# uberalex974/Reinforcement-Learning

Measured on AMD Instinct MI355X. Metric: env-steps/sec (whole node) at 32768 arenas; PPO wall-clock per 1M steps, higher is better.
Workload: dtype f32

## Files before the change

### include/rlgpu_core.h

```cpp
#ifndef RLGPU_CORE_H
#define RLGPU_CORE_H

#ifdef __cplusplus
extern "C" {
#endif

enum rlgpu_status {
    RLGPU_OK = 0,
    RLGPU_ERR_INVALID_ARG = -1,
    RLGPU_ERR_HIP = -2,
    RLGPU_ERR_OOM = -3,
    RLGPU_ERR_STATE = -4,
    RLGPU_ERR_UNSUPPORTED = -5
};

const char* rlgpu_last_error(void);

int rlgpu_abi_version(void);

int rlgpu_device_count(void);

#ifdef __cplusplus
}
#endif
#endif
```

### reinforcement-learning_amd/host/learner.cpp

```cpp
#include "learner.hpp"

#include <algorithm>
#include <chrono>
#include <cmath>
#include <cstdio>
#include <cstring>

#include "../csrc/common.hpp"
#include "../csrc/learner_kernels.hpp"

namespace {
constexpr int OBS = RLGPU_OBS, ACT = RLGPU_ACTIONS;
using clk = std::chrono::steady_clock;
double secs(clk::time_point a, clk::time_point b) { return std::chrono::duration<double>(b - a).count(); }

inline void hipCheck(hipError_t e, const char* what) {
    if (e != hipSuccess) throw rlgpu::Error(RLGPU_ERR_HIP, std::string(what) + ": " + hipGetErrorString(e));
}

inline uint64_t splitmix64(uint64_t x) {
    x += 0x9E3779B97F4A7C15ull;
    x = (x ^ (x >> 30)) * 0xBF58476D1CE4E5B9ull;
    x = (x ^ (x >> 27)) * 0x94D049BB133111EBull;
    return x ^ (x >> 31);
}
}

namespace RLGC {

EnvSetGPU::EnvSetGPU(const rlgpu_envset_config& cfg, hipStream_t stream) : stream_(stream) {
    RlgpuCheck(rlgpu_envset_create(&cfg, &h_), "EnvSet");
    RlgpuCheck(rlgpu_envset_buffers_get(h_, &state_), "EnvSet buffers");
}
EnvSetGPU::~EnvSetGPU() {
    if (h_) rlgpu_envset_destroy(h_);
}
void EnvSetGPU::StepFirstHalf(bool) { RlgpuCheck(rlgpu_envset_step_first_half(h_, stream_), "StepFirstHalf"); }
void EnvSetGPU::StepSecondHalf(const int32_t* d_actions, bool async) {
    RlgpuCheck(rlgpu_envset_step_second_half(h_, d_actions, stream_), "StepSecondHalf");
    if (!async) Sync();
}
void EnvSetGPU::Step(const int32_t* d_actions, const rlgpu_step_outputs* out) {
    RlgpuCheck(rlgpu_envset_step(h_, d_actions, 1, out, stream_), "EnvSet step");
}
void EnvSetGPU::Sync() { RlgpuCheck(rlgpu_envset_sync(h_, stream_), "Sync"); }
void EnvSetGPU::Reset() { RlgpuCheck(rlgpu_envset_reset(h_, stream_), "Reset"); }
void EnvSetGPU::ResetArenas(const uint8_t* d_mask) {
    RlgpuCheck(rlgpu_envset_reset_arenas(h_, d_mask, stream_), "ResetArena");
}

}

namespace GGL {

void WelfordStat::Increment(const float* xs, int64_t n) {
    for (int64_t i = 0; i < n; i++) {
        double delta = (double)xs[i] - mean;
        double deltaN = delta / (double)(count + 1);
        mean += deltaN;
        m2 += delta * deltaN * (double)count;
        count++;
    }
}
double WelfordStat::GetSTD() const {
    if (count < 2) return 1.0;
    double var = m2 / (double)(count - 1);
    if (var <= 0) var = 1.0;
    return std::sqrt(var);
}

void MomentsMeanStd(const double* m, float* out) {
    const double mean = m[0] / m[2];
    double var = (m[1] - m[0] * mean) / (m[2] - 1);
    if (!(var > 0)) var = 0;
    out[0] = (float)mean;
    out[1] = (float)std::sqrt(var);
}

std::vector<std::pair<int64_t, int64_t>> BatchRanges(int64_t expSize, int64_t batchSize, bool overbatching) {
    std::vector<std::pair<int64_t, int64_t>> out;
    if (expSize <= 0 || batchSize <= 0) return out;
    for (int64_t start = 0; start < expSize; start += batchSize) {
        int64_t end = start + batchSize;
        if (end + batchSize > expSize && overbatching) end = expSize;
        if (end > expSize || end - start <= 0) break;
        out.emplace_back(start, end);
        if (end == expSize) break;
    }
    return out;
}

template <class T>
void DevArray<T>::Reserve(int64_t n, hipStream_t s, bool keep) {
    if (n <= cap) return;
    const int64_t ncap = std::max<int64_t>(n, cap + cap / 2);
    T* q = nullptr;
    hipCheck(hipMalloc((void**)&q, (size_t)ncap * sizeof(T) + 16), "DevArray alloc");
    if (keep && p && cap > 0) hipCheck(hipMemcpyAsync(q, p, (size_t)cap * sizeof(T), hipMemcpyDeviceToDevice, s), "DevArray copy");
    if (p) {
        hipCheck(hipStreamSynchronize(s), "sync");
        (void)hipFree(p);
    }
    p = q;
    cap = ncap;
}
template <class T>
void DevArray<T>::Free() {
    if (p) (void)hipFree(p);
    p = nullptr;
    cap = 0;
}

void ExperienceBuffer::Allocate(int T_, int P_, int W_, bool rollout_outputs) {
    T = T_;
    P = P_;
    W = W_;
    auto A = [&](size_t bytes) {
        void* p = nullptr;
        hipCheck(hipMalloc(&p, bytes + 16), "ExperienceBuffer alloc");
        hipCheck(hipMemset(p, 0, bytes + 16), "ExperienceBuffer memset");
        allocs.push_back(p);
        return p;
    };
    const size_t TP = (size_t)T * P, T1P = (size_t)(T + 1) * P;
    const size_t OP = rollout_outputs ? TP : (size_t)P, O1P = rollout_outputs ? T1P : (size_t)P;
    v.obs = (float*)A(T1P * W * 4);
    v.masks = (uint8_t*)A(T1P * ACT);
    v.actions = (int32_t*)A(TP * 4);
    v.logp = (float*)A(TP * 4);
    v.rewards = (float*)A(TP * 4);
    v.terms = (int8_t*)A(TP);
    v.trunc_obs = (float*)A(OP * W * 4);
    v.values = (float*)A(O1P * 4);
    v.trunc_vals = (float*)A(OP * 4);
    v.adv = (float*)A(OP * 4);
    v.target = (float*)A(OP * 4);
    v.ret = (float*)A(OP * 4);
    v.T = T;
    v.P = P;
    v.obs_width = W;
}
void ExperienceBuffer::Free() {
    for (void* p : allocs) (void)hipFree(p);
    allocs.clear();
}

PPOLearnerGPU::PPOLearnerGPU(const rlgpu_ppo_config& cfg, hipStream_t stream) : stream_(stream) {
    RlgpuCheck(rlgpu_ppo_create(&cfg, &h_), "PPOLearner");
    float* params = nullptr;
    RlgpuCheck(rlgpu_ppo_buffers(h_, &params, &grads_, &nparams_), "PPOLearner buffers");
    hipCheck(hipMalloc((void**)&adv_stats_, 2 * sizeof(float)), "adv stats");
    hipCheck(hipMalloc((void**)&metrics_, RLGPU_NUM_METRICS * sizeof(float)), "metrics");
    hipCheck(hipMemset(metrics_, 0, RLGPU_NUM_METRICS * sizeof(float)), "metrics");
    RlgpuCheck(rlgpu_ppo_init_params(h_, cfg.seed, stream_), "init params");
}
PPOLearnerGPU::~PPOLearnerGPU() {
    if (adv_stats_) (void)hipFree(adv_stats_);
    if (metrics_) (void)hipFree(metrics_);
    if (h_) rlgpu_ppo_destroy(h_);
}
void PPOLearnerGPU::InferActions(const float* d_obs, const uint8_t* d_masks, int n, bool det, uint64_t step,
                                 int32_t* d_actions, float* d_logp, const uint8_t* d_old_rows) {
    if (d_old_rows)
        RlgpuCheck(rlgpu_ppo_infer_actions_mixed(h_, d_obs, d_masks, n, det, step, d_old_rows, d_actions, d_logp, stream_),
                   "InferActions (old version)");
    else
        RlgpuCheck(rlgpu_ppo_infer_actions(h_, d_obs, d_masks, n, det, step, d_actions, d_logp, stream_), "InferActions");
}
void PPOLearnerGPU::InferCritic(const float* d_obs, int64_t n, float* d_values) {
    RlgpuCheck(rlgpu_ppo_infer_critic(h_, d_obs, n, d_values, stream_), "InferCritic");
}
void PPOLearnerGPU::AdvantageStats(const float* d_adv, int64_t n) {
    RlgpuCheck(rlgpu_mean_std(d_adv, n, adv_stats_, stream_), "advantage stats");
}
void PPOLearnerGPU::Minibatch(const float* d_obs, const uint8_t* d_masks, const int32_t* d_actions, const float* d_logp,
                              const float* d_adv, const float* d_target, const int32_t* d_index, int64_t start, int n,
                              int64_t batch) {
    RlgpuCheck(rlgpu_ppo_minibatch(h_, d_obs, d_masks, d_actions, d_logp, d_adv, d_target, d_index, start, n, batch,
                                   adv_stats_, metrics_, stream_),
               "Learn minibatch");
    minibatches++;
}
void PPOLearnerGPU::OptimizerStep() { RlgpuCheck(rlgpu_ppo_optimizer_step(h_, metrics_, stream_), "optimizer step"); }

template <class T>
T* Learner::Alloc(size_t count) {
    void* p = nullptr;
    hipCheck(hipMalloc(&p, count * sizeof(T) + 16), "Learner alloc");
    allocs_.push_back(p);
    return (T*)p;
}
void Learner::Release(void* p) {
    for (auto& q : allocs_)
        if (q == p) {
            (void)hipFree(q);
            q = allocs_.back();
            allocs_.pop_back();
            return;
        }
}

Learner::Learner(const rlgpu_learner_config& cfg, const rlgpu_collective* coll, hipStream_t stream)
    : s_(stream), cfg_(cfg) {
    RLGPU_REQUIRE(cfg.num_arenas > 0 && cfg.rollout_len > 0 && cfg.epochs > 0 && cfg.mini_batch_size > 0,
                  "Learner: num_arenas, rollout_len, epochs and mini_batch_size must be > 0");
    RLGPU_REQUIRE(cfg.world >= 1 && cfg.rank >= 0 && cfg.rank < cfg.world, "Learner: bad rank / world");
    RLGPU_REQUIRE(cfg.world == 1 || (coll && coll->allreduce_sum_f32 && coll->allreduce_sum_f64 && coll->allgather_f32),
                  "Learner: world > 1 needs a complete rlgpu_collective");
    RLGPU_REQUIRE(cfg.return_samples >= 0, "Learner: return_samples must be >= 0");
    if (coll) {
        coll_ = *coll;
        hasColl_ = cfg.world > 1;
    }
    std::memset(&stats, 0, sizeof(stats));
    const int T = cfg.rollout_len, N = cfg.num_arenas, P = 4 * N;
    rlgpu_envset_config ec{};
    ec.num_arenas = N;
    ec.tick_skip = cfg.tick_skip;
    ec.action_delay = cfg.action_delay;
    ec.seed = cfg.seed * 1000003ull;
    ec.arena_offset = cfg.rank * N;
    ec.save_rewards = 1;
    ec.max_episode_steps = (int32_t)(cfg.max_episode_duration * (120.0f / (float)cfg.tick_skip));
    ec.mesh_tris = cfg.mesh_tris;
    ec.mesh_ntris = cfg.mesh_ntris;
    ec.mesh_objects = cfg.mesh_objects;
    ec.mesh_object_ntris = cfg.mesh_object_ntris;
    ec.rewards = cfg.rewards;
    ec.n_rewards = cfg.n_rewards;
    ec.terminals = cfg.terminals;
    ec.n_terminals = cfg.n_terminals;
    ec.arith = cfg.arith;
    env_ = new RLGC::EnvSetGPU(ec, s_);
    RlgpuCheck(rlgpu_envset_enable_step_metrics(env_->handle(), 1), "step metrics");
    RlgpuCheck(rlgpu_envset_set_output_only(env_->handle(), 1), "output-only rows");
    K_ = cfg.frame_stack > 1 ? cfg.frame_stack : 1;
    RLGPU_REQUIRE(K_ <= 16, "Learner: frame_stack must be <= 16");
    const int W = OBS * K_;
    rlgpu_ppo_config pc{};
    pc.obs_size = W;
    pc.num_actions = ACT;
    std::memcpy(pc.policy_layers, cfg.policy_layers, sizeof(pc.policy_layers));
    pc.n_policy_layers = cfg.n_policy_layers;
    std::memcpy(pc.critic_layers, cfg.critic_layers, sizeof(pc.critic_layers));
    pc.n_critic_layers = cfg.n_critic_layers;
    std::memcpy(pc.shared_layers, cfg.shared_layers, sizeof(pc.shared_layers));
    pc.n_shared_layers = cfg.n_shared_layers;
    RLGPU_REQUIRE(cfg.activation >= RLGPU_ACT_LEAKY_RELU && cfg.activation <= RLGPU_ACT_TANH,
                  "Learner: activation must be RLGPU_ACT_LEAKY_RELU, _RELU, _SIGMOID or _TANH");
    RLGPU_REQUIRE(cfg.no_layer_norm == 0 || cfg.no_layer_norm == 1, "Learner: no_layer_norm must be 0 or 1");
    RLGPU_REQUIRE(cfg.optimizer == RLGPU_OPT_ADAMW || cfg.optimizer == RLGPU_OPT_ADAM,
                  "Learner: optimizer must be RLGPU_OPT_ADAMW or RLGPU_OPT_ADAM");
    pc.layer_norm = cfg.no_layer_norm ? 0 : 1;
    pc.activation = cfg.activation;
    pc.leaky_slope = 0.01f;
    pc.policy_lr = cfg.policy_lr;
    pc.critic_lr = cfg.critic_lr;
    pc.beta1 = 0.9f;
    pc.beta2 = 0.999f;
    pc.eps = 1e-8f;
    pc.weight_decay = cfg.optimizer == RLGPU_OPT_ADAM ? 0.f : 1e-2f;
    pc.clip_range = cfg.clip_range;
    pc.entropy_scale = cfg.entropy_scale;
    pc.max_grad_norm = 0.5f;
    const int64_t TP = (int64_t)T * P;
    const int64_t rowsCap = cfg.experience_mode == RLGPU_EXP_TRAJECTORIES ? (int64_t)cfg.mini_batch_size : TP;
    pc.max_rows = (int32_t)std::max<int64_t>(std::min<int64_t>(cfg.mini_batch_size, rowsCap), std::min<int64_t>(P, 65536));
    pc.seed = cfg.seed;
    pc.sample_row_offset = (int64_t)cfg.rank * P;
    pc.train_gemm = cfg.train_gemm;
    pc.infer_fp16 = cfg.infer_fp16;
    pc.policy_temperature = cfg.policy_temperature;
    pc.mask_entropy = cfg.mask_entropy;
    ppo_ = new PPOLearnerGPU(pc, s_);
    if (hasColl_) {
        float* params = nullptr;
        float* g = nullptr;
        int64_t n = 0;
        RlgpuCheck(rlgpu_ppo_buffers(ppo_->handle(), &params, &g, &n), "buffers");
        if (cfg.rank != 0) hipCheck(hipMemsetAsync(params, 0, n * sizeof(float), s_), "broadcast");
        hipCheck(hipStreamSynchronize(s_), "sync");
        if (coll_.allreduce_sum_f32(coll_.user, params, n) != 0)
            throw rlgpu::Error(RLGPU_ERR_STATE, "Learner: parameter broadcast failed");
        RlgpuCheck(rlgpu_ppo_refresh_half(ppo_->handle(), s_), "refresh half");
    }
    if (trajMode()) {
        RLGPU_REQUIRE(ec.max_episode_steps > 0, "Learner: experience_mode 1 needs max_episode_duration > 0");
        TrajectoryStore& J = traj;
        J.maxLen = ec.max_episode_steps;
        const int64_t total = cfg.ts_per_itr > 0 ? cfg.ts_per_itr : (int64_t)T * P * cfg.world;
        J.tsPerItr = (total + cfg.world - 1) / cfg.world;
        const int64_t perStep = P;
        J.Tmax = cfg.experience_capacity > 0 ? cfg.experience_capacity
                                              : (int)(J.maxLen + 2 * ((J.tsPerItr + perStep - 1) / perStep) + 64);
        RLGPU_REQUIRE(J.Tmax > J.maxLen + 1, "Learner: experience_capacity must exceed the max episode length + 1");
        exp_.Allocate(J.Tmax, P, W, false);
        J.start = Alloc<int32_t>(P);
        J.len = Alloc<int32_t>(P);
        J.trnew = Alloc<int32_t>(P);
        J.counters = Alloc<int64_t>(lk::kTcCount);
        hipCheck(hipMemset(J.start, 0, (size_t)P * 4), "traj start");
        hipCheck(hipMemset(J.len, 0, (size_t)P * 4), "traj len");
        hipCheck(hipHostMalloc((void**)&J.hcounters, lk::kTcCount * sizeof(int64_t)), "pinned counters");
        if (K_ > 1) J.truncStage = Alloc<float>((size_t)P * W);
        const int64_t rc = 4 * (int64_t)P;
        for (auto* a : {&J.rp, &J.rstart, &J.rlen, &J.rcode, &J.rtidx}) a->Reserve(rc, s_);
        J.roff.Reserve(rc, s_);
        J.truncObs.Reserve(4 * (int64_t)P * W, s_);
    } else {
        exp_.Allocate(T, P, W);
    }
    const rlgpu_envset_buffers& st = env_->state();
    if (K_ > 1) {
        hist_ = Alloc<float>((size_t)(K_ - 1) * P * OBS);
        lk::stack_frames(st.obs, nullptr, nullptr, hist_, K_, P, OBS, exp_.v.obs, nullptr, s_);
    } else {
        hipCheck(hipMemcpyAsync(exp_.v.obs, st.obs, (size_t)P * OBS * 4, hipMemcpyDeviceToDevice, s_), "obs0");
    }
    hipCheck(hipMemcpyAsync(exp_.v.masks, st.action_masks, (size_t)P * ACT, hipMemcpyDeviceToDevice, s_), "masks0");
    std::vector<uint8_t> team(P);
    for (int k = 0; k < 2; k++) {
        oldRows_[k] = Alloc<uint8_t>(P);
        for (int p = 0; p < P; p++) team[p] = (uint8_t)(p % 2 == k);
        hipCheck(hipMemcpy(oldRows_[k], team.data(), P, hipMemcpyHostToDevice), "old rows");
    }
    trainRows_ = Alloc<int32_t>((size_t)TP / 2 + 1);
    perm_ = Alloc<int32_t>(TP);
    permRows_ = Alloc<int32_t>(TP);
    badv_ = Alloc<float>(TP);
    permCap_ = TP;
    truncRows_ = Alloc<int32_t>(TP);
    truncCount_ = Alloc<int32_t>(1);
    selBytes_ = lk::select_trunc_scratch_bytes(TP);
    selScratch_ = Alloc<char>(selBytes_);
    sampleIdx_ = Alloc<int64_t>((size_t)std::max(1, cfg.return_samples));
    samples_ = Alloc<float>((size_t)std::max(1, cfg.return_samples));
    ends_ = Alloc<int32_t>(P);
    hostEnds_.assign(P, -1);
    mom_ = (double*)Alloc<char>(4 * sizeof(double) + lk::moments_scratch_bytes());
    clipSums_ = Alloc<float>(2);
    hipCheck(hipStreamSynchronize(s_), "Learner init");
}

Learner::~Learner() {
    if (s_) (void)hipStreamSynchronize(s_);
    for (auto s : gs_) {
        (void)hipStreamSynchronize(s);
        (void)hipStreamDestroy(s);
    }
    for (auto e : gsEnd_) (void)hipEventDestroy(e);
    if (gsStart_) (void)hipEventDestroy(gsStart_);
    for (auto e : ev_) (void)hipEventDestroy(e);
    for (void* p : allocs_) (void)hipFree(p);
    if (truncObsC_) (void)hipFree(truncObsC_);
    if (truncValC_) (void)hipFree(truncValC_);
    if (traj.hcounters) (void)hipHostFree(traj.hcounters);
    for (auto* a : {&traj.rp, &traj.rstart, &traj.rlen, &traj.rcode, &traj.rtidx, &traj.cActs}) a->Free();
    traj.roff.Free();
    for (auto* a : {&traj.truncObs, &traj.truncVals, &traj.cObs, &traj.cLogp, &traj.cRews, &traj.cVals, &traj.cAdv,
                    &traj.cTarget, &traj.cRet})
        a->Free();
    traj.cMasks.Free();
    traj.cTerms.Free();
    exp_.Free();
    delete ppo_;
    delete env_;
}

int Learner::CollectGroups() const {
    const int want = cfg_.collect_groups > 0 ? cfg_.collect_groups : 1;
    if (want <= 1 || hook_ || K_ > 1 || trajMode() || !rlgpu_ppo_fused_infer(ppo_->handle(), 0)) return 1;
    if (cfg_.num_arenas % (4 * want) != 0) return 1;
    return want;
}

void Learner::CollectGrouped(int G) {
    const int T = exp_.T, P = exp_.P, W = exp_.W;
    const rlgpu_rollout_view& v = exp_.v;
    const uint8_t* old = OldRows();
    const int Na = cfg_.num_arenas / G, Pg = 4 * Na;
    if ((int)gs_.size() != G) {
        for (auto s : gs_) (void)hipStreamDestroy(s);
        for (auto e : gsEnd_) (void)hipEventDestroy(e);
        gs_.assign(G, nullptr);
        gsEnd_.assign(G, nullptr);
        for (int g = 0; g < G; g++) {
            hipCheck(hipStreamCreateWithFlags(&gs_[g], hipStreamNonBlocking), "group stream");
            hipCheck(hipEventCreateWithFlags(&gsEnd_[g], hipEventDisableTiming), "group event");
        }
        if (!gsStart_) hipCheck(hipEventCreateWithFlags(&gsStart_, hipEventDisableTiming), "group event");
    }
    if (envTiming_) EnsureEvents((size_t)2 * T * G);
    hipCheck(hipEventRecord(gsStart_, s_), "group start");
    for (int g = 0; g < G; g++) hipCheck(hipStreamWaitEvent(gs_[g], gsStart_, 0), "group wait");
    rlgpu_ppo* ph = ppo_->handle();
    rlgpu_envset* eh = env_->handle();
    for (int t = 0; t < T; t++) {
        const size_t r = (size_t)t * P;
        for (int g = 0; g < G; g++) {
            const size_t p0 = (size_t)g * Pg, a = r + p0;
            RlgpuCheck(rlgpu_ppo_infer_actions_rows(ph, v.obs + a * W, v.masks + a * ACT, Pg, (int64_t)p0,
                                                    cfg_.deterministic != 0, (uint64_t)stats.rng_step,
                                                    old ? old + p0 : nullptr, v.actions + a, v.logp + a, gs_[g]),
                       "InferActions (group)");
            rlgpu_step_outputs o{v.obs + (a + P) * OBS, v.masks + (a + P) * ACT, v.rewards + a, v.terms + a,
                                 v.trunc_obs + a * OBS};
            if (envTiming_) hipCheck(hipEventRecord(ev_[2 * ((size_t)t * G + g)], gs_[g]), "event");
            RlgpuCheck(rlgpu_envset_step_range(eh, g * Na, Na, v.actions + a, 1, &o, gs_[g]), "EnvSet step (group)");
            if (envTiming_) hipCheck(hipEventRecord(ev_[2 * ((size_t)t * G + g) + 1], gs_[g]), "event");
        }
        stats.rng_step++;
    }
    for (int g = 0; g < G; g++) {
        hipCheck(hipEventRecord(gsEnd_[g], gs_[g]), "group end");
        hipCheck(hipStreamWaitEvent(s_, gsEnd_[g], 0), "group join");
    }
}

void Learner::Collect() {
    if (trajMode()) {
        CollectTrajectories();
        return;
    }
    if (const int G = CollectGroups(); G > 1) {
        collectGroupsUsed_ = G;
        CollectGrouped(G);
        return;
    }
    collectGroupsUsed_ = 1;
    const int T = exp_.T, P = exp_.P, W = exp_.W;
    const rlgpu_rollout_view& v = exp_.v;
    if (envTiming_) EnsureEvents((size_t)2 * T);
    for (int t = 0; t < T; t++) {
        const size_t r = (size_t)t * P;
        ActAndStep(r, r + P, v.trunc_obs + r * OBS, v.trunc_obs + r * W, envTiming_ ? &ev_[2 * t] : nullptr);
    }
}

void Learner::ActAndStep(size_t row, size_t next, float* trunc, float* truncStacked, hipEvent_t* timing) {
    const int P = exp_.P, W = exp_.W;
    const rlgpu_rollout_view& v = exp_.v;
    const rlgpu_envset_buffers& st = env_->state();
    ppo_->InferActions(v.obs + row * W, v.masks + row * ACT, P, cfg_.deterministic != 0, (uint64_t)stats.rng_step,
                       v.actions + row, v.logp + row, OldRows());
    stats.rng_step++;
    rlgpu_step_outputs o{K_ > 1 ? nullptr : v.obs + next * OBS, v.masks + next * ACT, v.rewards + row, v.terms + row,
                         K_ > 1 ? nullptr : trunc};
    if (timing) hipCheck(hipEventRecord(timing[0], s_), "event");
    StepEnv(v.actions + row, o);
    if (timing) hipCheck(hipEventRecord(timing[1], s_), "event");
    if (K_ > 1) lk::stack_frames(st.obs, st.trunc_obs, v.terms + row, hist_, K_, P, OBS, v.obs + next * W, truncStacked, s_);
}

void Learner::EnsureEvents(size_t count) {
    if (ev_.size() >= count) return;
    for (auto e : ev_) (void)hipEventDestroy(e);
    ev_.assign(count, nullptr);
    for (auto& e : ev_) hipCheck(hipEventCreate(&e), "event");
}

void Learner::StepEnv(const int32_t* d_actions, const rlgpu_step_outputs& o) {
    if (!hook_) {
        env_->Step(d_actions, &o);
        return;
    }
    rlgpu_envset* e = env_->handle();
    const rlgpu_envset_buffers& st = env_->state();
    const int P = st.num_players;
    rlgpu_step_outputs pre{nullptr, nullptr, nullptr, o.terminals, nullptr};
    RlgpuCheck(rlgpu_envset_step(e, d_actions, 0, &pre, s_), "EnvSet step (hooked)");
    hipCheck(hipStreamSynchronize(s_), "sync");
    if (hook_(hookUser_, RLGPU_HOOK_AFTER_STEP) != 0)
        throw rlgpu::Error(RLGPU_ERR_STATE, std::string("Learner: step hook failed: ") + rlgpu_last_error());
    lk::host_step_finish(st.terminals, o.terminals, st.rewards, o.rewards, st.obs, st.trunc_obs, o.trunc_obs, P, OBS, s_);
    RlgpuCheck(rlgpu_envset_reset(e, s_), "EnvSet reset (hooked)");
    hipCheck(hipStreamSynchronize(s_), "sync");
    if (hook_(hookUser_, RLGPU_HOOK_AFTER_RESET) != 0)
        throw rlgpu::Error(RLGPU_ERR_STATE, std::string("Learner: step hook failed: ") + rlgpu_last_error());
    if (o.obs) hipCheck(hipMemcpyAsync(o.obs, st.obs, (size_t)P * OBS * 4, hipMemcpyDeviceToDevice, s_), "obs append");
    if (o.masks) hipCheck(hipMemcpyAsync(o.masks, st.action_masks, (size_t)P * ACT, hipMemcpyDeviceToDevice, s_), "mask append");
}

void Learner::Consume() {
    if (trajMode()) {
        ConsumeTrajectories();
        return;
    }
    const int T = exp_.T, P = exp_.P;
    const int64_t TP = (int64_t)T * P;
    const rlgpu_rollout_view& v = exp_.v;
    ppo_->InferCritic(v.obs, TP + P, v.values);
    lk::select_trunc(v.terms, TP, selScratch_, selBytes_, truncRows_, truncCount_, s_);
    int32_t ntr = 0;
    hipCheck(hipMemcpyAsync(&ntr, truncCount_, sizeof(int32_t), hipMemcpyDeviceToHost, s_), "trunc count");
    hipCheck(hipStreamSynchronize(s_), "sync");
    if (ntr > 0) {
        if (ntr > truncCap_) {
            if (truncObsC_) (void)hipFree(truncObsC_);
            if (truncValC_) (void)hipFree(truncValC_);
            truncCap_ = std::max<int64_t>(ntr, 2 * truncCap_);
            hipCheck(hipMalloc((void**)&truncObsC_, (size_t)truncCap_ * exp_.W * 4), "trunc obs");
            hipCheck(hipMalloc((void**)&truncValC_, (size_t)truncCap_ * 4), "trunc vals");
        }
        lk::gather_rows(v.trunc_obs, exp_.W, truncRows_, ntr, truncObsC_, s_);
        ppo_->InferCritic(truncObsC_, ntr, truncValC_);
        lk::scatter_f32(truncValC_, truncRows_, ntr, v.trunc_vals, s_);
    }
    const float std_ = (float)returnStat.GetSTD();
    RlgpuCheck(rlgpu_gae_rollout(v.rewards, v.terms, v.values, v.trunc_vals, v.values + TP, T, P, cfg_.gamma,
                                 cfg_.gae_lambda, std_, cfg_.reward_clip_range, v.adv, v.target, v.ret, nullptr, s_),
               "GAE");
    const int k = cfg_.return_samples;
    if (k <= 0) return;
    lk::last_ends(v.terms, T, P, ends_, s_);
    hipCheck(hipMemcpyAsync(hostEnds_.data(), ends_, (size_t)P * sizeof(int32_t), hipMemcpyDeviceToHost, s_), "ends");
    hipCheck(hipStreamSynchronize(s_), "sync");
    if (oldTeam_ >= 0)
        for (int p = oldTeam_; p < P; p += 2) hostEnds_[p] = -1;
    if (!hasColl_) {
        std::vector<int64_t> idx(k);
        int32_t m = 0;
        RlgpuCheck(rlgpu_sample_finished_rows(cfg_.seed, 0, stats.iteration, hostEnds_.data(), P, k, idx.data(), &m),
                   "return samples");
        FeedReturnStat(v.ret, idx, m);
        return;
    }
    const int world = cfg_.world;
    std::vector<float> mine((size_t)P), all((size_t)P * world);
    for (int p = 0; p < P; p++) mine[p] = (float)hostEnds_[p];
    if (coll_.allgather_f32(coll_.user, mine.data(), P, all.data()) != 0)
        throw rlgpu::Error(RLGPU_ERR_STATE, "Learner: trajectory-end all-gather failed");
    std::vector<int32_t> gends((size_t)P * world);
    for (size_t i = 0; i < gends.size(); i++) gends[i] = (int32_t)all[i];
    const int64_t GP = (int64_t)P * world;
    std::vector<int64_t> gidx(k), idx;
    std::vector<int32_t> slot;
    int32_t m = 0;
    RlgpuCheck(rlgpu_sample_finished_rows(cfg_.seed, 0, stats.iteration, gends.data(), (int32_t)GP, k, gidx.data(), &m),
               "return samples");
    for (int32_t i = 0; i < m; i++) {
        const int64_t t = gidx[i] / GP, gp = gidx[i] % GP;
        if (gp / P == cfg_.rank) {
            idx.push_back(t * P + (gp - (int64_t)cfg_.rank * P));
            slot.push_back(i);
        }
    }
    std::vector<float> hs(std::max<size_t>(idx.size(), 1));
    if (!idx.empty()) {
        hipCheck(hipMemcpyAsync(sampleIdx_, idx.data(), idx.size() * sizeof(int64_t), hipMemcpyHostToDevice, s_),
                 "sample idx");
        lk::gather_samples(v.ret, sampleIdx_, (int32_t)idx.size(), samples_, s_);
        hipCheck(hipMemcpyAsync(hs.data(), samples_, idx.size() * sizeof(float), hipMemcpyDeviceToHost, s_), "samples");
        hipCheck(hipStreamSynchronize(s_), "sync");
    }
    std::vector<double> draw((size_t)std::max(m, 1), 0.0);
    for (size_t j = 0; j < idx.size(); j++) draw[slot[j]] = (double)hs[j];
    if (m > 0 && coll_.allreduce_sum_f64(coll_.user, draw.data(), m) != 0)
        throw rlgpu::Error(RLGPU_ERR_STATE, "Learner: return-sample all-reduce failed");
    std::vector<float> got((size_t)std::max(m, 1));
    for (int32_t i = 0; i < m; i++) got[i] = (float)draw[i];
    returnStat.Increment(got.data(), m);
}

void Learner::FeedReturnStat(const float* d_ret, const std::vector<int64_t>& idx, int32_t m) {
    const int k = cfg_.return_samples;
    std::vector<float> hs((size_t)std::max(m, 1));
    if (m > 0) {
        hipCheck(hipMemcpyAsync(sampleIdx_, idx.data(), m * sizeof(int64_t), hipMemcpyHostToDevice, s_), "sample idx");
        lk::gather_samples(d_ret, sampleIdx_, m, samples_, s_);
        hipCheck(hipMemcpyAsync(hs.data(), samples_, m * sizeof(float), hipMemcpyDeviceToHost, s_), "samples");
        hipCheck(hipStreamSynchronize(s_), "sync");
    }
    if (hasColl_) {
        std::vector<float> mine((size_t)k + 1, 0.f), all((size_t)(k + 1) * cfg_.world);
        mine[0] = (float)m;
        std::copy(hs.begin(), hs.begin() + m, mine.begin() + 1);
        if (coll_.allgather_f32(coll_.user, mine.data(), k + 1, all.data()) != 0)
            throw rlgpu::Error(RLGPU_ERR_STATE, "Learner: return-sample all-gather failed");
        for (int r = 0; r < cfg_.world; r++) {
            const float* blk = all.data() + (size_t)r * (k + 1);
            returnStat.Increment(blk + 1, (int64_t)blk[0]);
        }
    } else {
        returnStat.Increment(hs.data(), m);
    }
}

void Learner::AllReduceGrads(int epoch, int batch) {
    if (!hasColl_ && !gradHook_) return;
    hipCheck(hipStreamSynchronize(s_), "sync");
    if (hasColl_ && coll_.allreduce_sum_f32(coll_.user, ppo_->grads(), ppo_->num_params()) != 0)
        throw rlgpu::Error(RLGPU_ERR_STATE, "Learner: gradient all-reduce failed");
    if (gradHook_ && gradHook_(gradHookUser_, ppo_->grads(), ppo_->num_params(), epoch, batch) != 0)
        throw rlgpu::Error(RLGPU_ERR_STATE, "Learner: the gradient hook failed");
}

void Learner::BatchAdvantageStats(const float* d_adv, const int32_t* d_idx, int64_t n) {
    if (!hasColl_) {
        if (d_idx) {
            NeedLearnRows(n, "the batch-advantage gather");
            lk::gather_f32(d_adv, d_idx, n, badv_, s_);
            ppo_->AdvantageStats(badv_, n);
        } else {
            ppo_->AdvantageStats(d_adv, n);
        }
        return;
    }
    lk::moments_f64(d_adv, d_idx, n, mom_ + 4, mom_, s_);
    double m[3];
    hipCheck(hipMemcpyAsync(m, mom_, sizeof(m), hipMemcpyDeviceToHost, s_), "moments");
    hipCheck(hipStreamSynchronize(s_), "sync");
    if (coll_.allreduce_sum_f64(coll_.user, m, 3) != 0)
        throw rlgpu::Error(RLGPU_ERR_STATE, "Learner: advantage-moment all-reduce failed");
    float st[2];
    MomentsMeanStd(m, st);
    hipCheck(hipMemcpyAsync(ppo_->adv_stats(), st, sizeof(st), hipMemcpyHostToDevice, s_), "adv stats");
    hipCheck(hipStreamSynchronize(s_), "sync");
}

void Learner::NeedLearnRows(int64_t n, const char* what) const {
    if (n > permCap_)
        throw rlgpu::Error(RLGPU_ERR_INVALID_ARG, std::string("Learner: ") + what + " needs " + std::to_string(n) +
                                                      " rows of learn scratch, " + std::to_string(permCap_) + " reserved");
}

void Learner::ReserveLearnRows(int64_t M) {
    if (M <= permCap_) return;
    const int64_t cap = std::max<int64_t>(M, permCap_ + permCap_ / 2);
    hipCheck(hipStreamSynchronize(s_), "sync");
    for (void* p : {(void*)perm_, (void*)permRows_, (void*)badv_}) Release(p);
    perm_ = Alloc<int32_t>(cap);
    permRows_ = Alloc<int32_t>(cap);
    badv_ = Alloc<float>(cap);
    permCap_ = cap;
}

void Learner::Learn() {
    const int T = exp_.T, P = exp_.P;
    rlgpu_rollout_view v = exp_.v;
    const bool rows = oldTeam_ >= 0 && !trajMode();
    int64_t M = rows ? (int64_t)T * (P / 2) : (int64_t)T * P;
    if (trajMode()) {
        M = traj.nrows;
        v.obs = traj.cObs.p;
        v.masks = traj.cMasks.p;
        v.actions = traj.cActs.p;
        v.logp = traj.cLogp.p;
        v.adv = traj.cAdv.p;
        v.target = traj.cTarget.p;
        if (M <= 0 && !hasColl_) return;
    }
    ReserveLearnRows(M);
    int64_t globalM = M * cfg_.world;
    if (trajMode() && hasColl_) {
        double m = (double)M;
        if (coll_.allreduce_sum_f64(coll_.user, &m, 1) != 0)
            throw rlgpu::Error(RLGPU_ERR_STATE, "Learner: batch-size all-reduce failed");
        globalM = (int64_t)m;
    }
    const int64_t batch = cfg_.batch_size > 0 ? cfg_.batch_size : globalM;
    const int64_t localBatch = cfg_.batch_size > 0 ? std::max<int64_t>(1, cfg_.batch_size / cfg_.world) : M;
    std::vector<std::pair<int64_t, int64_t>> trajRanges;
    if (trajMode() && hasColl_) {
        for (auto [g0, g1] : BatchRanges(globalM, batch, cfg_.overbatching != 0))
            trajRanges.emplace_back(globalM ? g0 * M / globalM : 0, globalM ? g1 * M / globalM : 0);
        if (trajRanges.empty()) trajRanges.emplace_back(0, 0);
    }
    if (rows) lk::train_rows(T, P, 1 - oldTeam_, trainRows_, s_);
    for (int epoch = 0; epoch < cfg_.epochs; epoch++) {
        NeedLearnRows(M, "the shuffle");
        RlgpuCheck(rlgpu_permutation(M, cfg_.seed + (uint64_t)cfg_.rank, (uint64_t)(stats.iteration * cfg_.epochs + epoch),
                                     perm_, s_),
                   "shuffle");
        const int32_t* order = perm_;
        if (rows) {
            NeedLearnRows(M, "the team row selection");
            if (M > (int64_t)T * (P / 2)) throw rlgpu::Error(RLGPU_ERR_INVALID_ARG, "Learner: team rows exceed T * P / 2");
            lk::compose(trainRows_, perm_, M, permRows_, s_);
            order = permRows_;
        }
        const auto ranges = trajMode() && hasColl_ ? trajRanges : BatchRanges(M, localBatch, cfg_.overbatching != 0);
        int bi = 0;
        for (auto [b0, b1] : ranges) {
            const bool whole = !rows && b0 == 0 && b1 == M;
            BatchAdvantageStats(v.adv, whole ? nullptr : order + b0, b1 - b0);
            for (int64_t s0 = b0; s0 < b1; s0 += cfg_.mini_batch_size) {
                const int n = (int)std::min<int64_t>(cfg_.mini_batch_size, b1 - s0);
                ppo_->Minibatch(v.obs, v.masks, v.actions, v.logp, v.adv, v.target, order, s0, n, batch);
            }
            AllReduceGrads(epoch, bi++);
            ppo_->OptimizerStep();
        }
    }
}

void Learner::FinishIteration() {
    const int T = exp_.T, P = exp_.P;
    const rlgpu_rollout_view& v = exp_.v;
    const size_t W = (size_t)exp_.W;
    const int64_t realPlayers = oldTeam_ < 0 ? P : P / 2;
    stats.iteration++;
    if (trajMode()) {
        stats.total_steps += (int64_t)traj.steps * realPlayers * cfg_.world;
        return;
    }
    hipCheck(hipMemcpyAsync(v.obs, v.obs + (size_t)T * P * W, (size_t)P * W * 4, hipMemcpyDeviceToDevice, s_), "obs");
    hipCheck(hipMemcpyAsync(v.masks, v.masks + (size_t)T * P * ACT, (size_t)P * ACT, hipMemcpyDeviceToDevice, s_), "masks");
    stats.total_steps += (int64_t)T * realPlayers * cfg_.world;
}

lk::TrajRecs TrajectoryStore::Records() const { return {rp.p, rstart.p, rlen.p, rcode.p, rtidx.p, roff.p}; }

void Learner::CollectTrajectories() {
    TrajectoryStore& J = traj;
    const int P = exp_.P, W = exp_.W, Tm = J.Tmax;
    const rlgpu_rollout_view& v = exp_.v;
    const rlgpu_envset_buffers& st = env_->state();
    const uint8_t* track = oldTeam_ >= 0 ? oldRows_[1 - oldTeam_] : nullptr;
    if (J.lastOldTeam >= 0) lk::traj_restart(oldRows_[J.lastOldTeam], P, (int)(J.step % Tm), J.start, J.len, s_);
    J.lastOldTeam = oldTeam_;
    hipCheck(hipMemsetAsync(J.counters, 0, lk::kTcCount * sizeof(int64_t), s_), "traj counters");
    J.firstStep = J.step;
    J.steps = 0;
    J.nrec = J.ntrunc = J.nrows = 0;
    for (;;) {
        const int64_t need = std::max(J.nrec, J.ntrunc) + P;
        if (J.rp.cap < need) {
// ... 399 lines not shown
```

### reinforcement-learning_amd/host/learner.hpp

```cpp
#pragma once
#include <hip/hip_runtime.h>

#include <cstdint>
#include <stdexcept>
#include <string>
#include <utility>
#include <vector>

#include "../../include/rlgpu_env.h"
#include "../../include/rlgpu_gae.h"
#include "../../include/rlgpu_learner.h"
#include "../../include/rlgpu_ppo.h"

namespace RLGC {

inline void RlgpuCheck(int st, const char* what) {
    if (st != RLGPU_OK) throw std::runtime_error(std::string(what) + ": " + rlgpu_last_error());
}

class EnvSetGPU {
public:
    EnvSetGPU(const rlgpu_envset_config& cfg, hipStream_t stream);
    ~EnvSetGPU();
    EnvSetGPU(const EnvSetGPU&) = delete;
    EnvSetGPU& operator=(const EnvSetGPU&) = delete;

    void StepFirstHalf(bool async = true);
    void StepSecondHalf(const int32_t* d_actions, bool async);
    void Step(const int32_t* d_actions, const rlgpu_step_outputs* out);
    void Sync();
    void Reset();
    void ResetArenas(const uint8_t* d_mask);

    rlgpu_envset* handle() const { return h_; }
    const rlgpu_envset_buffers& state() const { return state_; }

private:
    rlgpu_envset* h_ = nullptr;
    rlgpu_envset_buffers state_{};
    hipStream_t stream_;
};

}

namespace lk {
struct TrajRecs;
}

namespace GGL {

using RLGC::RlgpuCheck;

struct WelfordStat {
    int64_t count = 0;
    double mean = 0, m2 = 0;
    void Increment(const float* xs, int64_t n);
    double GetMean() const { return count < 2 ? 0.0 : mean; }
    double GetSTD() const;
};

void MomentsMeanStd(const double* m3, float* out2);

std::vector<std::pair<int64_t, int64_t>> BatchRanges(int64_t expSize, int64_t batchSize, bool overbatching);

struct ExperienceBuffer {
    int T = 0, P = 0, W = 0;
    rlgpu_rollout_view v{};
    std::vector<void*> allocs;
    void Allocate(int T, int P, int W, bool rollout_outputs = true);
    void Free();
};

template <class T>
struct DevArray {
    T* p = nullptr;
    int64_t cap = 0;
    void Reserve(int64_t n, hipStream_t s, bool keep = false);
    void Free();
};

struct TrajectoryStore {
    int Tmax = 0, maxLen = 0;
    int64_t tsPerItr = 0;
    int64_t step = 0;
    int64_t firstStep = 0;
    int steps = 0;
    int lastOldTeam = -1;
    int32_t *start = nullptr, *len = nullptr, *trnew = nullptr;
    int64_t* counters = nullptr;
    int64_t* hcounters = nullptr;
    DevArray<int32_t> rp, rstart, rlen, rcode, rtidx;
    DevArray<int64_t> roff;
    DevArray<float> truncObs, truncVals;
    DevArray<float> cObs, cLogp, cRews, cVals, cAdv, cTarget, cRet;
    DevArray<uint8_t> cMasks;
    DevArray<int32_t> cActs;
    DevArray<int8_t> cTerms;
    float* truncStage = nullptr;
    int64_t nrec = 0, ntrunc = 0, nrows = 0;
    lk::TrajRecs Records() const;
};

class PPOLearnerGPU {
public:
    PPOLearnerGPU(const rlgpu_ppo_config& cfg, hipStream_t stream);
    ~PPOLearnerGPU();
    PPOLearnerGPU(const PPOLearnerGPU&) = delete;
    PPOLearnerGPU& operator=(const PPOLearnerGPU&) = delete;

    void InferActions(const float* d_obs, const uint8_t* d_masks, int n, bool deterministic, uint64_t step,
                      int32_t* d_actions, float* d_logp, const uint8_t* d_old_rows = nullptr);
    void InferCritic(const float* d_obs, int64_t n, float* d_values);
    void AdvantageStats(const float* d_adv, int64_t n);
    void Minibatch(const float* d_obs, const uint8_t* d_masks, const int32_t* d_actions, const float* d_logp,
                   const float* d_adv, const float* d_target, const int32_t* d_index, int64_t start, int n,
                   int64_t batch);
    void OptimizerStep();
    int64_t minibatches = 0;

    rlgpu_ppo* handle() const { return h_; }
    float* grads() const { return grads_; }
    int64_t num_params() const { return nparams_; }
    float* adv_stats() const { return adv_stats_; }
    float* metrics() const { return metrics_; }

private:
    rlgpu_ppo* h_ = nullptr;
    hipStream_t stream_;
    float* grads_ = nullptr;
    int64_t nparams_ = 0;
    float* adv_stats_ = nullptr;
    float* metrics_ = nullptr;
};

class Learner {
public:
    Learner(const rlgpu_learner_config& cfg, const rlgpu_collective* coll, hipStream_t stream);
    ~Learner();
    Learner(const Learner&) = delete;
    Learner& operator=(const Learner&) = delete;

    void Collect();
    void Consume();
    void Learn();
    void FinishIteration();
    rlgpu_learner_report Iterate();
    void Start(int64_t iterations);

    void SetOldTeam(int team) { oldTeam_ = team; }
    void SetGradHook(rlgpu_grad_hook_fn fn, void* user) {
        gradHook_ = fn;
        gradHookUser_ = user;
    }
    void SetStepHook(rlgpu_step_hook_fn fn, void* user) {
        hook_ = fn;
        hookUser_ = user;
    }
    void SetEnvTiming(bool on) { envTiming_ = on; }

    const rlgpu_learner_config& config() const { return cfg_; }
    RLGC::EnvSetGPU& env() { return *env_; }
    PPOLearnerGPU& ppo() { return *ppo_; }
    ExperienceBuffer& exp() { return exp_; }
    rlgpu_learner_stats stats;
    WelfordStat returnStat;

private:
    void StepEnv(const int32_t* d_actions, const rlgpu_step_outputs& o);
    void ActAndStep(size_t row, size_t next, float* trunc, float* truncStacked, hipEvent_t* timing);
    void EnsureEvents(size_t count);
    void AllReduceGrads(int epoch, int batch);
    void BatchAdvantageStats(const float* d_adv, const int32_t* d_idx, int64_t n);
    void CollectTrajectories();
    void ConsumeTrajectories();
    void FeedReturnStat(const float* d_ret, const std::vector<int64_t>& idx, int32_t m);
    bool trajMode() const { return cfg_.experience_mode == RLGPU_EXP_TRAJECTORIES; }
    hipStream_t s_;
    rlgpu_learner_config cfg_;
    rlgpu_collective coll_{};
    bool hasColl_ = false;
    RLGC::EnvSetGPU* env_ = nullptr;
    PPOLearnerGPU* ppo_ = nullptr;
    ExperienceBuffer exp_;
    int oldTeam_ = -1;
    bool envTiming_ = false;
    rlgpu_step_hook_fn hook_ = nullptr;
    void* hookUser_ = nullptr;
    rlgpu_grad_hook_fn gradHook_ = nullptr;
    void* gradHookUser_ = nullptr;
    int K_ = 1;
    float* hist_ = nullptr;
    std::vector<hipEvent_t> ev_;
    std::vector<hipStream_t> gs_;
    std::vector<hipEvent_t> gsEnd_;
    hipEvent_t gsStart_ = nullptr;
    int CollectGroups() const;
    int collectGroupsUsed_ = 1;
    void CollectGrouped(int G);
    uint8_t* oldRows_[2] = {nullptr, nullptr};
    const uint8_t* OldRows() const { return oldTeam_ >= 0 ? oldRows_[oldTeam_] : nullptr; }
    int32_t* trainRows_ = nullptr;
    int32_t* perm_ = nullptr;
    int32_t* permRows_ = nullptr;
    float* badv_ = nullptr;
    int64_t permCap_ = 0;
    void NeedLearnRows(int64_t n, const char* what) const;
    void ReserveLearnRows(int64_t M);
    int32_t* truncRows_ = nullptr;
    int32_t* truncCount_ = nullptr;
    void* selScratch_ = nullptr;
    size_t selBytes_ = 0;
    float* truncObsC_ = nullptr;
    float* truncValC_ = nullptr;
    int64_t truncCap_ = 0;
    int64_t* sampleIdx_ = nullptr;
    float* samples_ = nullptr;
    int32_t* ends_ = nullptr;
    std::vector<int32_t> hostEnds_;
    double* mom_ = nullptr;
    float* clipSums_ = nullptr;
  public:
    TrajectoryStore traj;
  private:
    std::vector<void*> allocs_;
    template <class T>
    T* Alloc(size_t count);
    void Release(void* p);
};

}
```

Baseline: 1.981 million.

## Partition CUs across collect-group streams and enable two groups by default

Group collection streams are now created with hipExtStreamCreateWithCUMask, so each group's inference and env-step kernels run on a disjoint, XCD-balanced set of CUs on gfx950. Grouped collection is also turned on automatically with two groups when there are at least 4096 arenas. The intent is to let the two group pipelines overlap without competing for the same CUs, cutting serialization and interference during rollout. The cost is that each group can use only half the device, which may hurt kernels that could otherwise fill all CUs. Debug APIs and a probe kernel are added to check which CUs each stream's work lands on.

```diff
diff --git a/include/rlgpu_core.h b/include/rlgpu_core.h
--- a/include/rlgpu_core.h
+++ b/include/rlgpu_core.h
@@ -1,5 +1,7 @@
 #ifndef RLGPU_CORE_H
 #define RLGPU_CORE_H
+
+#include <stdint.h>
 
 #ifdef __cplusplus
 extern "C" {
@@ -20,6 +22,13 @@
 
 int rlgpu_device_count(void);
 
+int rlgpu_cu_partition(int32_t cu_count, int32_t groups, uint32_t* masks, int32_t words);
+
+int rlgpu_debug_cu_stream_create(int32_t groups, int32_t group, void** stream);
+int rlgpu_debug_cu_stream_mask(void* stream, uint32_t* mask, int32_t words);
+int rlgpu_debug_cu_stream_destroy(void* stream);
+int rlgpu_debug_cu_probe(void* stream, uint32_t* d_out, int32_t n_workgroups, int32_t hold_us);
+
 #ifdef __cplusplus
 }
 #endif
diff --git a/reinforcement-learning_amd/csrc/cu_probe.hip b/reinforcement-learning_amd/csrc/cu_probe.hip
--- /dev/null
+++ b/reinforcement-learning_amd/csrc/cu_probe.hip
@@ -0,0 +1,32 @@
+#include "common.hpp"
+
+namespace {
+
+constexpr int kHwRegHwId = 4, kHwRegXccId = 20;
+constexpr int getreg(int id, int offset, int size) { return id | (offset << 6) | ((size - 1) << 11); }
+constexpr unsigned kMaxHoldUs = 2000;
+
+__global__ void __launch_bounds__(64) cu_probe_kernel(uint32_t* out, int n, unsigned hold_ticks) {
+    asm volatile("" ::: "v255", "a255");
+    const uint32_t hw = __builtin_amdgcn_s_getreg(getreg(kHwRegHwId, 0, 32));
+    const uint32_t xcc = __builtin_amdgcn_s_getreg(getreg(kHwRegXccId, 0, 4));
+    const unsigned long long t0 = wall_clock64();
+    for (int i = 0; i < (1 << 20) && wall_clock64() - t0 < hold_ticks; i++) __builtin_amdgcn_s_sleep(8);
+    const int w = (int)blockIdx.x;
+    if (w < n && threadIdx.x < 4) {
+        const uint32_t v = threadIdx.x == 0 ? xcc : threadIdx.x == 1 ? (hw >> 13) & 7u : threadIdx.x == 2 ? (hw >> 8) & 15u : hw;
+        out[(size_t)w * 4 + threadIdx.x] = v;
+    }
+}
+
+}
+
+extern "C" int rlgpu_debug_cu_probe(void* stream, uint32_t* d_out, int32_t n_workgroups, int32_t hold_us) {
+    return rlgpu::guarded([&] {
+        RLGPU_REQUIRE(d_out && n_workgroups > 0 && n_workgroups <= 65536, "rlgpu_debug_cu_probe: 1 .. 65536 workgroups");
+        RLGPU_REQUIRE(hold_us >= 0 && (unsigned)hold_us <= kMaxHoldUs, "rlgpu_debug_cu_probe: hold of 0 .. 2000 us");
+        hipLaunchKernelGGL(cu_probe_kernel, dim3((unsigned)n_workgroups), dim3(64), 0, rlgpu::as_stream(stream), d_out,
+                           (int)n_workgroups, (unsigned)hold_us * 100u);
+        RLGPU_CHECK_HIP(hipGetLastError());
+    });
+}
diff --git a/reinforcement-learning_amd/host/cu_partition.cpp b/reinforcement-learning_amd/host/cu_partition.cpp
--- /dev/null
+++ b/reinforcement-learning_amd/host/cu_partition.cpp
@@ -0,0 +1,92 @@
+#include "cu_partition.hpp"
+
+#include <cstring>
+
+#include "../../include/rlgpu_core.h"
+#include "../csrc/common.hpp"
+
+namespace rlgpu {
+
+int cu_partition_group(int k, int groups) {
+    if (groups != 2 && groups != 4 && groups != 8 && groups != 16) return -1;
+    if (k < 0 || k >= kPartitionCUs) return -1;
+    const int b = k;
+    const int g = ((b >> 3) & 1) | (((b >> 4) & 1) << 1) | ((((b >> 2) ^ (b >> 5)) & 1) << 2) |
+                  ((((b >> 1) ^ (b >> 6)) & 1) << 3);
+    return g & (groups - 1);
+}
+
+bool cu_partition_masks(int cu_count, int groups, std::vector<uint32_t>& masks) {
+    if (cu_count != kPartitionCUs || cu_partition_group(0, groups) < 0) return false;
+    std::vector<uint32_t> m((size_t)groups * kPartitionWords, 0u);
+    for (int k = 0; k < kPartitionCUs; k++)
+        m[(size_t)cu_partition_group(k, groups) * kPartitionWords + k / 32] |= 1u << (k % 32);
+    const int want = kPartitionCUs / kPartitionXCDs / groups;
+    for (int g = 0; g < groups; g++) {
+        int inter[kPartitionXCDs] = {}, block[kPartitionXCDs] = {};
+        for (int k = 0; k < kPartitionCUs; k++)
+            if (m[(size_t)g * kPartitionWords + k / 32] >> (k % 32) & 1u) {
+                inter[k % kPartitionXCDs]++;
+                block[k / (kPartitionCUs / kPartitionXCDs)]++;
+            }
+        for (int x = 0; x < kPartitionXCDs; x++)
+            if (inter[x] != want || block[x] != want) return false;
+    }
+    masks.swap(m);
+    return true;
+}
+
+hipError_t cu_partition_stream(int groups, int group, hipStream_t* out) {
+    *out = nullptr;
+    int dev = 0;
+    hipError_t e = hipGetDevice(&dev);
+    if (e != hipSuccess) return e;
+    hipDeviceProp_t p;
+    e = hipGetDeviceProperties(&p, dev);
+    if (e != hipSuccess) return e;
+    std::vector<uint32_t> masks;
+    if (std::strncmp(p.gcnArchName, "gfx950", 6) != 0 || group < 0 || group >= groups ||
+        !cu_partition_masks(p.multiProcessorCount, groups, masks))
+        return hipErrorNotSupported;
+    return hipExtStreamCreateWithCUMask(out, kPartitionWords, masks.data() + (size_t)group * kPartitionWords);
+}
+
+}
+
+extern "C" int rlgpu_cu_partition(int32_t cu_count, int32_t groups, uint32_t* masks, int32_t words) {
+    return rlgpu::guarded([&] {
+        RLGPU_REQUIRE(masks && words == rlgpu::kPartitionWords, "rlgpu_cu_partition: masks of 8 words each");
+        std::vector<uint32_t> m;
+        if (!rlgpu::cu_partition_masks(cu_count, groups, m))
+            throw rlgpu::Error(RLGPU_ERR_UNSUPPORTED, "rlgpu_cu_partition: no balanced partition of " +
+                                                          std::to_string(cu_count) + " CUs into " +
+                                                          std::to_string(groups) + " groups");
+        std::memcpy(masks, m.data(), m.size() * sizeof(uint32_t));
+    });
+}
+
+extern "C" int rlgpu_debug_cu_stream_create(int32_t groups, int32_t group, void** stream) {
+    return rlgpu::guarded([&] {
+        RLGPU_REQUIRE(stream, "rlgpu_debug_cu_stream_create: stream is null");
+        hipStream_t s = nullptr;
+        const hipError_t e = rlgpu::cu_partition_stream(groups, group, &s);
+        if (e == hipErrorNotSupported)
+            throw rlgpu::Error(RLGPU_ERR_UNSUPPORTED, "rlgpu_debug_cu_stream_create: no balanced partition of this device into " +
+                                                          std::to_string(groups) + " groups");
+        RLGPU_CHECK_HIP(e);
+        *stream = s;
+    });
+}
+
+extern "C" int rlgpu_debug_cu_stream_mask(void* stream, uint32_t* mask, int32_t words) {
+    return rlgpu::guarded([&] {
+        RLGPU_REQUIRE(mask && words > 0, "rlgpu_debug_cu_stream_mask: mask of at least one word");
+        RLGPU_CHECK_HIP(hipExtStreamGetCUMask(rlgpu::as_stream(stream), (uint32_t)words, mask));
+    });
+}
+
+extern "C" int rlgpu_debug_cu_stream_destroy(void* stream) {
+    return rlgpu::guarded([&] {
+        if (stream) RLGPU_CHECK_HIP(hipStreamDestroy(rlgpu::as_stream(stream)));
+    });
+}
diff --git a/reinforcement-learning_amd/host/cu_partition.hpp b/reinforcement-learning_amd/host/cu_partition.hpp
--- /dev/null
+++ b/reinforcement-learning_amd/host/cu_partition.hpp
@@ -0,0 +1,19 @@
+#pragma once
+#include <hip/hip_runtime_api.h>
+
+#include <cstdint>
+#include <vector>
+
+namespace rlgpu {
+
+constexpr int kPartitionCUs = 256;
+constexpr int kPartitionXCDs = 8;
+constexpr int kPartitionWords = kPartitionCUs / 32;
+
+int cu_partition_group(int k, int groups);
+
+bool cu_partition_masks(int cu_count, int groups, std::vector<uint32_t>& masks);
+
+hipError_t cu_partition_stream(int groups, int group, hipStream_t* out);
+
+}
diff --git a/reinforcement-learning_amd/host/learner.cpp b/reinforcement-learning_amd/host/learner.cpp
--- a/reinforcement-learning_amd/host/learner.cpp
+++ b/reinforcement-learning_amd/host/learner.cpp
@@ -8,6 +8,7 @@
 
 #include "../csrc/common.hpp"
 #include "../csrc/learner_kernels.hpp"
+#include "cu_partition.hpp"
 
 namespace {
 constexpr int OBS = RLGPU_OBS, ACT = RLGPU_ACTIONS;
@@ -367,11 +368,44 @@
     delete env_;
 }
 
+constexpr int kAutoCollectGroups = 2;
+constexpr int kAutoCollectArenas = 4096;
+
 int Learner::CollectGroups() const {
-    const int want = cfg_.collect_groups > 0 ? cfg_.collect_groups : 1;
+    const int want = cfg_.collect_groups > 0                   ? cfg_.collect_groups
+                     : cfg_.num_arenas >= kAutoCollectArenas ? kAutoCollectGroups
+                                                             : 1;
     if (want <= 1 || hook_ || K_ > 1 || trajMode() || !rlgpu_ppo_fused_infer(ppo_->handle(), 0)) return 1;
     if (cfg_.num_arenas % (4 * want) != 0) return 1;
     return want;
+}
+
+bool Learner::EnsureGroupStreams(int G) {
+    if ((int)gs_.size() == G) return true;
+    if (gsRefused_ == G) return false;
+    for (auto s : gs_) {
+        (void)hipStreamSynchronize(s);
+        (void)hipStreamDestroy(s);
+    }
+    for (auto e : gsEnd_) (void)hipEventDestroy(e);
+    gs_.clear();
+    gsEnd_.clear();
+    std::vector<hipStream_t> ss;
+    for (int g = 0; g < G; g++) {
+        hipStream_t s = nullptr;
+        if (rlgpu::cu_partition_stream(G, g, &s) != hipSuccess) {
+            (void)hipGetLastError();
+            for (auto x : ss) (void)hipStreamDestroy(x);
+            gsRefused_ = G;
+            return false;
+        }
+        ss.push_back(s);
+    }
+    gs_ = ss;
+    gsEnd_.assign(G, nullptr);
+    for (int g = 0; g < G; g++) hipCheck(hipEventCreateWithFlags(&gsEnd_[g], hipEventDisableTiming), "group event");
+    if (!gsStart_) hipCheck(hipEventCreateWithFlags(&gsStart_, hipEventDisableTiming), "group event");
+    return true;
 }
 
 void Learner::CollectGrouped(int G) {
@@ -379,17 +413,6 @@
     const rlgpu_rollout_view& v = exp_.v;
     const uint8_t* old = OldRows();
     const int Na = cfg_.num_arenas / G, Pg = 4 * Na;
-    if ((int)gs_.size() != G) {
-        for (auto s : gs_) (void)hipStreamDestroy(s);
-        for (auto e : gsEnd_) (void)hipEventDestroy(e);
-        gs_.assign(G, nullptr);
-        gsEnd_.assign(G, nullptr);
-        for (int g = 0; g < G; g++) {
-            hipCheck(hipStreamCreateWithFlags(&gs_[g], hipStreamNonBlocking), "group stream");
-            hipCheck(hipEventCreateWithFlags(&gsEnd_[g], hipEventDisableTiming), "group event");
-        }
-        if (!gsStart_) hipCheck(hipEventCreateWithFlags(&gsStart_, hipEventDisableTiming), "group event");
-    }
     if (envTiming_) EnsureEvents((size_t)2 * T * G);
     hipCheck(hipEventRecord(gsStart_, s_), "group start");
     for (int g = 0; g < G; g++) hipCheck(hipStreamWaitEvent(gs_[g], gsStart_, 0), "group wait");
@@ -422,7 +445,7 @@
         CollectTrajectories();
         return;
     }
-    if (const int G = CollectGroups(); G > 1) {
+    if (const int G = CollectGroups(); G > 1 && EnsureGroupStreams(G)) {
         collectGroupsUsed_ = G;
         CollectGrouped(G);
         return;
diff --git a/reinforcement-learning_amd/host/learner.hpp b/reinforcement-learning_amd/host/learner.hpp
--- a/reinforcement-learning_amd/host/learner.hpp
+++ b/reinforcement-learning_amd/host/learner.hpp
@@ -194,7 +194,9 @@
     std::vector<hipStream_t> gs_;
     std::vector<hipEvent_t> gsEnd_;
     hipEvent_t gsStart_ = nullptr;
+    int gsRefused_ = 0;
     int CollectGroups() const;
+    bool EnsureGroupStreams(int G);
     int collectGroupsUsed_ = 1;
     void CollectGrouped(int G);
     uint8_t* oldRows_[2] = {nullptr, nullptr};
diff --git a/reinforcement-learning_amd/rlgpu/partition.py b/reinforcement-learning_amd/rlgpu/partition.py
--- /dev/null
+++ b/reinforcement-learning_amd/rlgpu/partition.py
@@ -0,0 +1,63 @@
+import ctypes
+
+import numpy as np
+
+from . import _lib
+
+WORDS = 8
+
+
+def masks(cu_count, groups):
+    out = np.zeros((max(groups, 1), WORDS), np.uint32)
+    L = _lib.lib()
+    L.rlgpu_cu_partition.argtypes = [ctypes.c_int32, ctypes.c_int32, ctypes.c_void_p, ctypes.c_int32]
+    _lib.check(L.rlgpu_cu_partition(cu_count, groups, out.ctypes.data, WORDS), "rlgpu_cu_partition")
+    return out
+
+
+def mask_bits(mask):
+    return [32 * w + b for w, x in enumerate(np.asarray(mask, np.uint32).tolist()) for b in range(32) if x >> b & 1]
+
+
+class PartitionStream:
+
+    def __init__(self, groups, group):
+        import torch
+        L = _lib.lib()
+        L.rlgpu_debug_cu_stream_create.argtypes = [ctypes.c_int32, ctypes.c_int32, ctypes.POINTER(ctypes.c_void_p)]
+        h = ctypes.c_void_p()
+        _lib.check(L.rlgpu_debug_cu_stream_create(groups, group, ctypes.byref(h)), "rlgpu_debug_cu_stream_create")
+        self._h = h
+        self.stream = torch.cuda.ExternalStream(h.value)
+
+    def mask(self):
+        out = np.zeros(WORDS, np.uint32)
+        L = _lib.lib()
+        L.rlgpu_debug_cu_stream_mask.argtypes = [ctypes.c_void_p, ctypes.c_void_p, ctypes.c_int32]
+        _lib.check(L.rlgpu_debug_cu_stream_mask(self._h, out.ctypes.data, WORDS), "rlgpu_debug_cu_stream_mask")
+        return out
+
+    def close(self):
+        if self._h:
+            L = _lib.lib()
+            L.rlgpu_debug_cu_stream_destroy.argtypes = [ctypes.c_void_p]
+            self.stream.synchronize()
+            _lib.check(L.rlgpu_debug_cu_stream_destroy(self._h), "rlgpu_debug_cu_stream_destroy")
+            self._h = None
+
+    def __del__(self):
+        try:
+            self.close()
+        except Exception:
+            pass
+
+
+def probe(stream, n_workgroups, hold_us=200):
+    import torch
+    out = torch.full((n_workgroups, 4), -1, dtype=torch.int32, device="cuda")
+    torch.cuda.current_stream().synchronize()
+    L = _lib.lib()
+    L.rlgpu_debug_cu_probe.argtypes = [ctypes.c_void_p, ctypes.c_void_p, ctypes.c_int32, ctypes.c_int32]
+    _lib.check(L.rlgpu_debug_cu_probe(_lib.stream_ptr(stream), _lib.ptr(out), n_workgroups, hold_us), "rlgpu_debug_cu_probe")
+    (stream if stream is not None else torch.cuda.current_stream()).synchronize()
+    return out.cpu().numpy().view(np.uint32).astype(np.int64)
```

After: 2.049 million, median of 6. +3.4%, better.
